# OvO1111/JointImageGeneration

Measured on AMD Instinct MI355X. Metric: sampled voxels/sec @50 DDIM steps, 128^3 mask + 512^2x256 CT, higher is better.
Workload: dtype bf16; 1 GPU; C5 full GuideGen volume per GPU: CCDM 128^3 K=14 250 steps -> LDM 256 slices x (cond-encode + 50 DDIM @4x64x64 + AE decode 512^2); volumes_per_gpu=1, ccdm_steps=250, ddim_steps=50, slices=256, parallelism=replicas x1 (one volume per GPU, no collective), weights=random-init (seed recipe)

## Files before the change

include/guidegen_hip.h:

```cpp
#ifndef GUIDEGEN_HIP_H
#define GUIDEGEN_HIP_H

#include <stdint.h>

#ifdef __cplusplus
extern "C" {
#endif

typedef enum {
    GG_OK = 0,
    GG_ERR_BAD_SHAPE = -1,
    GG_ERR_BAD_DTYPE = -2,
    GG_ERR_UNSUPPORTED = -3,
    GG_ERR_WORKSPACE_TOO_SMALL = -4,
    GG_ERR_HIP = -5
} gg_status;

typedef enum { GG_BF16 = 0, GG_F32 = 1 } gg_dtype;

const char *gg_last_error(void);
int gg_version(void);

typedef struct {
    int32_t N, D, H, W;
// ... 9 lines not shown
    int32_t prologue_act;
    int32_t path_hint;
    const void *src1;
    const void *src2;
    const void *weight;
    const float *bias;
    int64_t bias_stride;
    const void *residual;
    void *out;
    const float *gn_scale;
    const float *gn_shift;
    void *workspace;
    int64_t workspace_bytes;
    void *reserved_ptr;
    int64_t *gn_acc;
    float *ddim_x;
    const float *ddim_scalars;
    float *ddim_pred_x0;
    void *ddim_unet_in;
    int64_t ddim_unet_in_stride;
    int32_t epilogue_geglu;
    int32_t pro_c_logical;
    const int64_t *pro_acc1;
    const int64_t *pro_acc2;
    const float *pro_gamma;
    const float *pro_beta;
    float pro_eps;
    int32_t skip_C1, skip_C2;
    int32_t reserved_tail;
    const void *skip_src1;
    const void *skip_src2;
    const void *skip_weight;
    const int32_t *post_xt;
    int32_t *post_labels_out;
    const float *post_scalars;
    const float *post_E;
    uint64_t post_philox_seed;
    const int64_t *post_philox_offset_dev;
    void *post_onehot_out;
    int64_t post_onehot_stride;
    int32_t post_draw;
    int32_t reserved_tail2;
    const uint64_t *post_philox_seeds;
    int64_t post_rows_per_sample;
} gg_conv_desc;

int64_t gg_conv_packed_weight_bytes(int32_t Cout, int32_t Cin_pad, int32_t ntaps);
int gg_conv_pack_weight(const float *w_f32, int32_t Cout, int32_t Cin, int32_t Cin_pad, int32_t ntaps,
                        void *packed_bf16, void *stream);
int64_t gg_conv_workspace_bytes(const gg_conv_desc *desc);
int gg_conv_fuses_prologue(const gg_conv_desc *desc);
int gg_conv_fuses_posterior(const gg_conv_desc *desc);
int gg_conv_runs_halo_tile(const gg_conv_desc *desc);
int gg_conv_emits_stats(const gg_conv_desc *desc);
int gg_conv_prologue_from_acc(const gg_conv_desc *desc);
int gg_conv_fuses_skip(const gg_conv_desc *desc);
int gg_conv_fuses_ddim(const gg_conv_desc *desc);
int gg_conv_forward(const gg_conv_desc *desc, void *stream);

int64_t gg_groupnorm_workspace_bytes(int32_t N, int64_t S, int32_t C);
int gg_groupnorm_stats(const void *src1, int32_t C1, const void *src2, int32_t C2, int32_t N, int64_t S,
                       int32_t C_logical, const float *gamma, const float *beta, float eps,
                       float *scale_out, float *shift_out, void *workspace, int64_t workspace_bytes, void *stream);
int gg_groupnorm_apply(const void *src1, int32_t C1, const void *src2, int32_t C2, int32_t N, int64_t S,
                       const float *scale, const float *shift, int32_t act, void *out, void *stream);
int gg_groupnorm_fused_supported(int64_t S, int32_t C1, int32_t C2, int32_t C_logical);
int gg_groupnorm_fused(const void *src1, int32_t C1, const void *src2, int32_t C2, int32_t N, int64_t S, int32_t C_logical,
                       const float *gamma, const float *beta, float eps, int32_t act, void *out, void *stream);
int gg_groupnorm_apply_acc(const void *src1, int32_t C1, const int64_t *acc1, const void *src2, int32_t C2, const int64_t *acc2,
                           int32_t N, int64_t S, int32_t C_logical, const float *gamma, const float *beta, float eps,
                           int32_t act, void *out, void *stream);

int gg_groupnorm_scale_shift_acc(const int64_t *acc1, int32_t stripes1, int32_t C1, const int64_t *acc2, int32_t stripes2, int32_t C2,
                                 int32_t N, int64_t S, int32_t C_logical, const float *gamma, const float *beta, float eps,
                                 float *scale_out, float *shift_out, void *stream);

int gg_resample2x(const void *src, int32_t dtype, int32_t N, int32_t D, int32_t H, int32_t W, int32_t C_pad, int32_t C_logical,
                  int32_t resample_d, int32_t mode, const float *scale, const float *shift, int32_t act, void *dst, void *stream);
int gg_film_fold(float *scale, float *shift, int32_t coef_stride, int32_t N, int32_t C, const float *film, int64_t film_stride, void *stream);

typedef struct {
    int32_t N, heads, head_dim;
    int32_t Tq, Tkv;
    int64_t ldq, hsq, ldk, hsk, ldv, hsv, ldo, hso;
    float scale;
    int32_t reserved;
    const void *q, *k, *v;
    void *out;
    void *workspace;
    int64_t workspace_bytes;
} gg_attention_desc;
int gg_attention_forward(const gg_attention_desc *desc, void *stream);
int64_t gg_attention_workspace_bytes(const gg_attention_desc *desc);
int gg_attention_plan(const gg_attention_desc *desc, int32_t plan[4]);

int gg_layernorm(const void *x, int64_t rows, int32_t C, const float *gamma, const float *beta, float eps,
                 void *out, void *stream);
int gg_geglu(const void *h, int64_t rows, int32_t inner, void *out, void *stream);
int gg_add(const void *a, const void *b, int64_t n, void *out, void *stream);

int gg_linear_f32(const float *in, int32_t M, int32_t I, const float *W, const float *b, int32_t O,
                  int32_t act_in, float *out, int64_t out_stride, void *stream);
int gg_timestep_embedding(const float *t, int32_t M, int32_t dim, float max_period, float *out, void *stream);

int gg_nchw_f32_to_cl_bf16(const float *src, int32_t N, int32_t C, int64_t S, void *dst, int32_t C_pad,
                           int32_t c_offset, int32_t zero_fill, void *stream);
// ... 73 lines not shown
```

jointimagegeneration_amd/_lib.py:

```python
from __future__ import annotations

import ctypes as C
import os

_HERE = os.path.dirname(os.path.abspath(__file__))
LIB_PATH = os.path.join(_HERE, "csrc", "libguidegen_hip.so")

GG_BF16, GG_F32 = 0, 1

vp, i32, i64, u64, f32 = C.c_void_p, C.c_int32, C.c_int64, C.c_uint64, C.c_float


class ConvDesc(C.Structure):
    _fields_ = [
        ("N", i32), ("D", i32), ("H", i32), ("W", i32),
        ("C1", i32), ("C2", i32), ("Cout", i32), ("Cout_pad", i32),
        ("kd", i32), ("kh", i32), ("kw", i32), ("stride", i32), ("pad", i32), ("upsample", i32),
        ("Do", i32), ("Ho", i32), ("Wo", i32), ("out_dtype", i32), ("prologue_act", i32), ("path_hint", i32),
        ("src1", vp), ("src2", vp), ("weight", vp), ("bias", vp), ("bias_stride", i64),
        ("residual", vp), ("out", vp), ("gn_scale", vp), ("gn_shift", vp), ("workspace", vp), ("workspace_bytes", i64), ("reserved_ptr", vp), ("gn_acc", vp),
        ("ddim_x", vp), ("ddim_scalars", vp), ("ddim_pred_x0", vp), ("ddim_unet_in", vp), ("ddim_unet_in_stride", i64),
        ("epilogue_geglu", i32), ("pro_c_logical", i32), ("pro_acc1", vp), ("pro_acc2", vp), ("pro_gamma", vp), ("pro_beta", vp),
        ("pro_eps", f32), ("skip_C1", i32), ("skip_C2", i32), ("reserved_tail", i32), ("skip_src1", vp), ("skip_src2", vp), ("skip_weight", vp),
        ("post_xt", vp), ("post_labels_out", vp), ("post_scalars", vp), ("post_E", vp), ("post_philox_seed", C.c_uint64),
        ("post_philox_offset_dev", vp), ("post_onehot_out", vp), ("post_onehot_stride", i64), ("post_draw", i32), ("reserved_tail2", i32),
        ("post_philox_seeds", vp), ("post_rows_per_sample", i64),
    ]


class AttentionDesc(C.Structure):
    _fields_ = [
        ("N", i32), ("heads", i32), ("head_dim", i32), ("Tq", i32), ("Tkv", i32),
        ("ldq", i64), ("hsq", i64), ("ldk", i64), ("hsk", i64), ("ldv", i64), ("hsv", i64), ("ldo", i64), ("hso", i64),
        ("scale", f32), ("reserved", i32),
        ("q", vp), ("k", vp), ("v", vp), ("out", vp), ("workspace", vp), ("workspace_bytes", i64),
    ]


SIGNATURES = {
    "gg_last_error": (C.c_char_p, []),
    "gg_version": (C.c_int, []),
    "gg_conv_packed_weight_bytes": (i64, [i32, i32, i32]),
    "gg_conv_pack_weight": (C.c_int, [vp, i32, i32, i32, i32, vp, vp]),
    "gg_conv_forward": (C.c_int, [C.POINTER(ConvDesc), vp]),
    "gg_conv_workspace_bytes": (i64, [C.POINTER(ConvDesc)]),
    "gg_conv_fuses_prologue": (C.c_int, [C.POINTER(ConvDesc)]),
    "gg_conv_runs_halo_tile": (C.c_int, [C.POINTER(ConvDesc)]),
    "gg_conv_emits_stats": (C.c_int, [C.POINTER(ConvDesc)]),
    "gg_conv_prologue_from_acc": (C.c_int, [C.POINTER(ConvDesc)]),
    "gg_conv_fuses_skip": (C.c_int, [C.POINTER(ConvDesc)]),
    "gg_conv_fuses_ddim": (C.c_int, [C.POINTER(ConvDesc)]),
    "gg_conv_fuses_posterior": (C.c_int, [C.POINTER(ConvDesc)]),
    "gg_groupnorm_workspace_bytes": (i64, [i32, i64, i32]),
    "gg_groupnorm_stats": (C.c_int, [vp, i32, vp, i32, i32, i64, i32, vp, vp, f32, vp, vp, vp, i64, vp]),
    "gg_groupnorm_apply": (C.c_int, [vp, i32, vp, i32, i32, i64, vp, vp, i32, vp, vp]),
    "gg_groupnorm_apply_acc": (C.c_int, [vp, i32, vp, vp, i32, vp, i32, i64, i32, vp, vp, f32, i32, vp, vp]),
    "gg_groupnorm_fused_supported": (C.c_int, [i64, i32, i32, i32]),
    "gg_groupnorm_fused": (C.c_int, [vp, i32, vp, i32, i32, i64, i32, vp, vp, f32, i32, vp, vp]),
    "gg_groupnorm_scale_shift_acc": (C.c_int, [vp, i32, i32, vp, i32, i32, i32, i64, i32, vp, vp, f32, vp, vp, vp]),
    "gg_attention_forward": (C.c_int, [C.POINTER(AttentionDesc), vp]),
    "gg_attention_workspace_bytes": (i64, [C.POINTER(AttentionDesc)]),
    "gg_attention_plan": (C.c_int, [C.POINTER(AttentionDesc), C.POINTER(i32)]),
    "gg_layernorm": (C.c_int, [vp, i64, i32, vp, vp, f32, vp, vp]),
    "gg_geglu": (C.c_int, [vp, i64, i32, vp, vp]),
    "gg_add": (C.c_int, [vp, vp, i64, vp, vp]),
    "gg_linear_f32": (C.c_int, [vp, i32, i32, vp, vp, i32, i32, vp, i64, vp]),
    "gg_timestep_embedding": (C.c_int, [vp, i32, i32, f32, vp, vp]),
    "gg_nchw_f32_to_cl_bf16": (C.c_int, [vp, i32, i32, i64, vp, i32, i32, i32, vp]),
    "gg_cl_to_nchw_f32": (C.c_int, [vp, i32, i32, i32, i64, i32, vp, vp]),
    "gg_ccdm_posterior_sample": (C.c_int, [vp, i32, i32, vp, vp, u64, vp, i32, vp, i32, i64, vp, vp, vp, i32, vp]),
    "gg_ccdm_posterior_sample_seeds": (C.c_int, [vp, i32, i32, vp, vp, vp, i64, vp, i32, vp, i32, i64, vp, vp, vp, i32, vp]),
    "gg_labels_to_onehot": (C.c_int, [vp, i64, i32, vp, i32, vp]),
    "gg_ddim_step": (C.c_int, [vp, vp, i32, vp, vp, i64, i32, vp, vp, i32, vp]),
    "gg_minmax_normalise": (C.c_int, [vp, i64, vp, vp, vp]),
    "gg_ddpm_step": (C.c_int, [vp, vp, i32, vp, vp, i64, i32, vp, i32, vp]),
    "gg_inpaint_blend": (C.c_int, [vp, vp, vp, i32, vp, vp, i64, i32, vp, i32, vp]),
    "gg_vq_nearest": (C.c_int, [vp, i32, vp, i32, i32, i64, vp, vp, i32, vp]),
    "gg_ddim_step_vq": (C.c_int, [vp, vp, i32, vp, vp, i32, vp, i32, i64, i32, vp, vp, vp, i32, vp]),
    "gg_label_confusion": (C.c_int, [vp, i32, vp, i32, i64, i32, vp, vp, vp]),
    "gg_volume_views_cl": (C.c_int, [vp, i32, i32, i32, i32, i32, i64, i64, vp, vp, vp, i32, vp]),
    "gg_relu_cl": (C.c_int, [vp, i32, i64, vp]),
    "gg_lpips_tap_workspace_bytes": (i64, [i32, i32, i32, i32, i32]),
    "gg_lpips_tap": (C.c_int, [vp, vp, i32, i32, i32, i32, i32, vp, vp, vp, vp, vp, i32, vp, i64, vp]),
    "gg_unfold_cl": (C.c_int, [vp, i32, i32, i32, i32, i32, i32, vp, i32, i32, i32, i32, i32, i32, i32, vp]),
    "gg_fold_weighted_cl": (C.c_int, [vp, i32, vp, vp, vp, i32, i32, i32, i32, i32, i32, i32, i32, i32, vp]),
    "gg_lincomb4": (C.c_int, [vp, vp, vp, vp, f32, f32, f32, f32, f32, i64, vp, vp]),
    "gg_conv_forward_f32": (C.c_int, [C.POINTER(ConvDesc), vp]),
    "gg_groupnorm_f32": (C.c_int, [vp, i32, vp, i32, i32, i64, i32, vp, vp, f32, i32, vp, vp, vp]),
    "gg_attention_forward_f32": (C.c_int, [C.POINTER(AttentionDesc), vp]),
    "gg_groupnorm_f32_film": (C.c_int, [vp, i32, i32, i64, i32, vp, vp, f32, vp, i64, i32, vp, vp, vp]),
    "gg_resample2x": (C.c_int, [vp, i32, i32, i32, i32, i32, i32, i32, i32, i32, vp, vp, i32, vp, vp]),
    "gg_film_fold": (C.c_int, [vp, vp, i32, i32, i32, vp, i64, vp]),
    "gg_mask_to_cond_slice": (C.c_int, [vp, i32, i32, i32, i32, i32, i32, i32, i32, vp, vp, i32, vp, vp]),
    "gg_mask_to_cond_slices": (C.c_int, [vp, i32, i32, i32, i32, i32, i32, i32, vp, i32, vp, vp, vp, i32, vp]),
    "gg_minmax_normalise_scatter": (C.c_int, [vp, i32, i64, vp, vp, i32, vp, i32, i32, vp, vp]),
    "gg_ubench_mfma_bf16": (C.c_int, [i32, i32, i32, vp, C.POINTER(C.c_double), vp]),
    "gg_ubench_stream_copy": (C.c_int, [vp, vp, i64, vp]),
}

_lib = None
# ... 27 lines not shown
```

jointimagegeneration_amd/csrc/gg_conv.h:

```cpp
#pragma once
#include "gg_common.h"

struct ConvParams {
    int N, D, H, W, C1, C2, Cout, Cout_pad;
    int kd, kh, kw, stride, pad, upsample;
    int Do, Ho, Wo, out_dtype, prologue_act;
    int path_hint;
    int nchunk1, nchunk, ntaps;
    long long M;
    long long bias_stride;
    const bf16_t *src1, *src2, *weight, *residual;
    const float *bias, *gn_scale, *gn_shift;
    void *out;
    float *ws;
    int splitk;
    long long *gn_acc;
    float *ddim_x, *ddim_pred_x0;
    const float *ddim_scalars;
    bf16_t *ddim_unet_in;
    long long ddim_unet_in_stride;
    unsigned mg_osp, mg_ohw, mg_wo;
    int epi_geglu;
    const long long *pro_acc1, *pro_acc2;
    const float *pro_gamma, *pro_beta;
    float pro_eps;
    int pro_clog;
    const bf16_t *skip_src1, *skip_src2, *skip_weight;
    int skip_C1, skip_C2;
    const int *post_xt;
    int *post_labels_out;
    const float *post_scalars, *post_E;
    unsigned long long post_seed;
    const long long *post_offset_dev;
    bf16_t *post_onehot_out;
    long long post_onehot_stride;
    int post_draw;
    const unsigned long long *post_seeds;
    long long post_rows_per_sample;
};

#define GG_BOX_HINT_GENERIC 10
#define GG_BOX_HINT_SPEC_ONLY 11

#define GG_ACC_SUM_SCALE 268435456.0f
#define GG_ACC_SQ_SCALE 1048576.0f
#ifndef GG_ACC_STRIPES
#define GG_ACC_STRIPES 1
#endif
#define GG_ACC_STRIPES_HALO 32

__device__ __forceinline__ int swz64(int row, int chunk) { return chunk ^ ((row >> 1) & 2); }


__device__ __forceinline__ float gg_row16_sum(float x)
{
    x += __builtin_bit_cast(float, __builtin_amdgcn_mov_dpp(__builtin_bit_cast(int, x), 0xB1, 0xF, 0xF, true));
    x += __builtin_bit_cast(float, __builtin_amdgcn_mov_dpp(__builtin_bit_cast(int, x), 0x4E, 0xF, 0xF, true));
    x += __builtin_bit_cast(float, __builtin_amdgcn_mov_dpp(__builtin_bit_cast(int, x), 0x141, 0xF, 0xF, true));
    x += __builtin_bit_cast(float, __builtin_amdgcn_mov_dpp(__builtin_bit_cast(int, x), 0x140, 0xF, 0xF, true));
    return x;
}
```

jointimagegeneration_amd/csrc/gg_conv.hip:

```cpp
#include "gg_conv.h"
#include <stdlib.h>

template <int NT, int PF, int PRO>
__global__ __launch_bounds__(256) void conv_gather_kernel(const ConvParams p)
{
    constexpr int BM = 128;
    constexpr int XBYTES = BM * 64;
    constexpr int WBYTES = NT * 32 * 64;
    constexpr int STAGE = XBYTES + WBYTES;
    constexpr int WITER = (NT * 128 + 255) / 256;
    __shared__ __attribute__((aligned(16))) char smem[2 * STAGE];

    const int tid = threadIdx.x;
    const int lane = tid & 63;
    const int wave = tid >> 6;
    const long long m0 = (long long)blockIdx.x * BM;
    const int g0 = blockIdx.y * NT;

    const int xq = tid & 3;
    int bn[2], bd[2], bh[2], bw[2];
    bool rv[2];
    const bf16_t *rb1[2], *rb2[2];
    const unsigned osp = (unsigned)(p.Do * p.Ho * p.Wo);
    const unsigned ohw = (unsigned)(p.Ho * p.Wo);
// ... 513 lines not shown
    }
}

__global__ void conv_pack_weight_kernel(const float *__restrict__ w, int Cout, int Cin, int Cin_pad, int ntaps,
                                        int Cout_pad, bf16_t *__restrict__ dst)
{
    const int nchunk = Cin_pad >> 5;
    const long long total = (long long)Cout_pad * ntaps * Cin_pad;
    for (long long i = (long long)blockIdx.x * blockDim.x + threadIdx.x; i < total;
         i += (long long)gridDim.x * blockDim.x) {
        int cil = (int)(i & 31);
        int col = (int)((i >> 5) & 31);
        long long t = i >> 10;
        int chunk = (int)(t % nchunk);
        t /= nchunk;
        int tap = (int)(t % ntaps);
        int g = (int)(t / ntaps);
        int co = g * 32 + col, ci = chunk * 32 + swz64(col, cil >> 3) * 8 + (cil & 7);
        float v = 0.f;
        if (co < Cout && ci < Cin) v = w[((long long)co * Cin + ci) * ntaps + tap];
        dst[i] = (bf16_t)v;
    }
}

extern "C" int64_t gg_conv_packed_weight_bytes(int32_t Cout, int32_t Cin_pad, int32_t ntaps)
{
    int64_t cp = ((int64_t)Cout + 31) / 32 * 32;
    return cp * ntaps * Cin_pad * 2;
}

extern "C" int gg_conv_pack_weight(const float *w, int32_t Cout, int32_t Cin, int32_t Cin_pad, int32_t ntaps,
                                   void *packed, void *stream)
{
    if (Cin_pad % 32 || Cin > Cin_pad || Cout <= 0 || ntaps <= 0) GG_FAIL(GG_ERR_BAD_SHAPE, "pack_weight: bad shape");
    int Cout_pad = (Cout + 31) / 32 * 32;
    long long total = (long long)Cout_pad * ntaps * Cin_pad;
    int blocks = (int)((total + 255) / 256);
    if (blocks > 4096) blocks = 4096;
    hipLaunchKernelGGL(conv_pack_weight_kernel, dim3(blocks), dim3(256), 0, (hipStream_t)stream, w, Cout, Cin, Cin_pad,
                       ntaps, Cout_pad, (bf16_t *)packed);
    GG_CHECK_LAUNCH();
    return GG_OK;
}

int gg_conv_halo_try(const ConvParams &p, hipStream_t stream);
bool gg_conv_halo_prefers_separate_norm(const ConvParams &p);
#ifndef GG_HALO_SEPARATE_NORM
#define GG_HALO_SEPARATE_NORM 1
#endif
int gg_conv_box_try(const ConvParams &p, hipStream_t stream);
bool gg_conv_box_fuses_prologue(const ConvParams &p);
int gg_conv_tiny_plan(long long M, int Cout_pad, int KS, int prologue_act);
int gg_conv_tiny_launch(const ConvParams &p, hipStream_t stream);

static int launch_splitk_reduce(const ConvParams &p, hipStream_t stream, bool cap_blocks)
{
    long long blocks = (p.M * (p.Cout_pad / 4) + 255) / 256;
    if (cap_blocks && blocks > 2048) blocks = 2048;
    hipLaunchKernelGGL(conv_splitk_reduce_kernel, dim3((unsigned)blocks), dim3(256), 0, stream, p);
    GG_CHECK_LAUNCH();
    return GG_OK;
}

template <int NT>
static int launch_gather(const ConvParams &p, hipStream_t stream)
{
    dim3 grid((unsigned)((p.M + 127) / 128), (unsigned)(p.Cout_pad / (32 * NT)), (unsigned)p.splitk);
    if (p.prologue_act)
        hipLaunchKernelGGL((conv_gather_kernel<NT, (NT <= 2 ? 4 : 2), 1>), grid, dim3(256), 0, stream, p);
    else
        hipLaunchKernelGGL((conv_gather_kernel<NT, (NT <= 2 ? 4 : 2), 0>), grid, dim3(256), 0, stream, p);
    GG_CHECK_LAUNCH();
    return p.splitk > 1 ? launch_splitk_reduce(p, stream, true) : GG_OK;
}

static int launch_gather_nt(int NT, const ConvParams &p, hipStream_t stream)
{
    switch (NT) {
        case 5: return launch_gather<5>(p, stream);
        case 4: return launch_gather<4>(p, stream);
        case 3: return launch_gather<3>(p, stream);
        case 2: return launch_gather<2>(p, stream);
        default: return launch_gather<1>(p, stream);
    }
}

struct GatherPlan { int NT, splitk; };
static GatherPlan plan_gather(long long M, int Cout_pad, int KS)
{
    const int G = Cout_pad / 32;
    int NT = (G % 4 == 0) ? 4 : (G % 5 == 0) ? 5 : (G % 3 == 0) ? 3 : (G % 2 == 0) ? 2 : 1;
    const long long mb = (M + 127) / 128;
    int splitk = 1;
    constexpr int k_target = 512, k_minsteps = 8;
    if (mb * (G / NT) < 192) {
        if (G % 2 == 0 && NT > 2 && mb * (G / 2) <= 1024) NT = 2;
        if (mb * (G / NT) < 192 && NT > 1) NT = 1;
        long long blocks = mb * (G / NT);
        long long want = (k_target + blocks - 1) / blocks;
        long long maxs = KS / k_minsteps > 0 ? KS / k_minsteps : 1;
        splitk = (int)(want < maxs ? want : maxs);
        if (splitk < 1) splitk = 1;
        if (splitk > 64) splitk = 64;
    }
    return {NT, splitk};
}

static int plan_gather5(long long M, int C1, int C2, int Cout_pad, int ntaps)
{
    if (C1 % 160 || C2 % 160) return 0;
    const long long blocks = ((M + 63) / 64) * (Cout_pad / 32);
    if (blocks >= 4096) return 0;
    const int KS5 = ((C1 + C2) / 160) * ntaps;
    constexpr int g5_target = 320, g5_minsteps = 5;
    long long sk = (g5_target + blocks - 1) / blocks;
    long long maxs = KS5 / g5_minsteps > 0 ? KS5 / g5_minsteps : 1;
    if (sk > maxs) sk = maxs;
    if (sk < 1) sk = 1;
    if (sk > 32) sk = 32;
    return (int)sk;
}

extern "C" int64_t gg_conv_workspace_bytes(const gg_conv_desc *d)
{
    if (!d || d->epilogue_geglu) return 0;
    long long M = (long long)d->N * d->Do * d->Ho * d->Wo;
    int KS = d->kd * d->kh * d->kw * ((d->C1 + d->C2) / 32);
    if (int tsk = gg_conv_tiny_plan(M, d->Cout_pad, KS, d->prologue_act)) return tsk > 1 ? (int64_t)tsk * M * d->Cout_pad * 4 : 0;
    if (int s5 = plan_gather5(M, d->C1, d->C2, d->Cout_pad, d->kd * d->kh * d->kw)) return s5 > 1 ? (int64_t)s5 * M * d->Cout_pad * 4 : 0;
    GatherPlan pl = plan_gather(M, d->Cout_pad, KS);
    return pl.splitk > 1 ? (int64_t)pl.splitk * M * d->Cout_pad * 4 : 0;
}

static void fill_params(const gg_conv_desc *d, ConvParams &p)
{
    p.N = d->N; p.D = d->D; p.H = d->H; p.W = d->W; p.C1 = d->C1; p.C2 = d->C2; p.Cout = d->Cout; p.Cout_pad = d->Cout_pad;
    p.kd = d->kd; p.kh = d->kh; p.kw = d->kw; p.stride = d->stride; p.pad = d->pad; p.upsample = d->upsample;
    p.Do = d->Do; p.Ho = d->Ho; p.Wo = d->Wo; p.out_dtype = d->out_dtype; p.prologue_act = d->prologue_act; p.path_hint = d->path_hint;
    p.nchunk1 = d->C1 / 32; p.nchunk = (d->C1 + d->C2) / 32; p.ntaps = d->kd * d->kh * d->kw;
    p.M = (long long)d->N * d->Do * d->Ho * d->Wo;
    p.bias_stride = d->bias_stride;
    p.src1 = (const bf16_t *)d->src1; p.src2 = (const bf16_t *)d->src2; p.weight = (const bf16_t *)d->weight;
    p.residual = (const bf16_t *)d->residual; p.bias = d->bias; p.gn_scale = d->gn_scale; p.gn_shift = d->gn_shift;
    p.out = d->out;
    p.ws = nullptr;
    p.splitk = 1;
    p.gn_acc = (long long *)d->gn_acc;
    p.ddim_x = d->ddim_x; p.ddim_pred_x0 = d->ddim_pred_x0; p.ddim_scalars = d->ddim_scalars;
    p.ddim_unet_in = (bf16_t *)d->ddim_unet_in; p.ddim_unet_in_stride = d->ddim_unet_in_stride;
    p.epi_geglu = d->epilogue_geglu;
    p.pro_acc1 = (const long long *)d->pro_acc1; p.pro_acc2 = (const long long *)d->pro_acc2; p.pro_gamma = d->pro_gamma; p.pro_beta = d->pro_beta;
    p.pro_eps = d->pro_eps; p.pro_clog = d->pro_c_logical;
    if (d->gn_scale || d->gn_shift || !d->prologue_act) p.pro_acc1 = p.pro_acc2 = nullptr;
    p.skip_src1 = (const bf16_t *)d->skip_src1; p.skip_src2 = (const bf16_t *)d->skip_src2; p.skip_weight = (const bf16_t *)d->skip_weight;
    p.skip_C1 = d->skip_C1; p.skip_C2 = d->skip_C2;
    p.post_xt = d->post_xt; p.post_labels_out = d->post_labels_out; p.post_scalars = d->post_scalars; p.post_E = d->post_E;
    p.post_seed = d->post_philox_seed; p.post_offset_dev = (const long long *)d->post_philox_offset_dev;
    p.post_onehot_out = (bf16_t *)d->post_onehot_out; p.post_onehot_stride = d->post_onehot_stride; p.post_draw = d->post_draw;
    p.post_seeds = (const unsigned long long *)d->post_philox_seeds; p.post_rows_per_sample = d->post_rows_per_sample;
    p.mg_osp = gg_magic_u32(p.M, d->Do * d->Ho * d->Wo); p.mg_ohw = gg_magic_u32(p.M, d->Ho * d->Wo); p.mg_wo = gg_magic_u32(p.M, d->Wo);
}

static bool halo_try_dry(const ConvParams &p) { return gg_conv_halo_try(p, (hipStream_t)-1) == GG_OK; }
static bool box_try_dry(const ConvParams &p) { return gg_conv_box_try(p, (hipStream_t)-1) == GG_OK; }
static bool desc_channels_ok(const gg_conv_desc *d) { return d && d->C1 > 0 && d->C1 % 32 == 0 && d->C2 % 32 == 0 && d->Cout_pad % 32 == 0; }

static int take_splitk_workspace(const gg_conv_desc *d, ConvParams &p, int splitk)
{
    if (splitk > 1) {
        const long long need = (long long)splitk * p.M * p.Cout_pad * 4;
        if (!d->workspace || d->workspace_bytes < need)
            GG_FAIL(GG_ERR_WORKSPACE_TOO_SMALL, "conv: split-K needs %lld workspace bytes (gg_conv_workspace_bytes), got %lld", need, (long long)d->workspace_bytes);
        p.ws = (float *)d->workspace;
    }
    p.splitk = splitk;
    return GG_OK;
}

extern "C" int gg_conv_runs_halo_tile(const gg_conv_desc *d)
{
    if (!desc_channels_ok(d) || d->epilogue_geglu) return 0;
    ConvParams p;
    fill_params(d, p);
    return halo_try_dry(p) ? 1 : 0;
}

extern "C" int gg_conv_fuses_prologue(const gg_conv_desc *d)
{
    if (!desc_channels_ok(d) || d->epilogue_geglu) return 0;
    ConvParams p;
    fill_params(d, p);
    if (halo_try_dry(p)) return (GG_HALO_SEPARATE_NORM && d->path_hint == 0 && gg_conv_halo_prefers_separate_norm(p)) ? 0 : 1;
    if (box_try_dry(p)) return gg_conv_box_fuses_prologue(p) ? 1 : 0;
    return 0;
}

bool gg_conv_box_emits_stats(const ConvParams &p);
bool gg_conv_box_prologue_from_acc(const ConvParams &p);
bool gg_conv_halo_fuses_posterior(const ConvParams &p);

extern "C" int gg_conv_fuses_posterior(const gg_conv_desc *d)
{
    if (!desc_channels_ok(d) || d->epilogue_geglu || d->residual || d->out_dtype != GG_F32 || d->gn_acc ||
        d->ddim_x || d->skip_C1) return 0;
    ConvParams p;
    fill_params(d, p);
    return gg_conv_halo_fuses_posterior(p) ? 1 : 0;
}

extern "C" int gg_conv_prologue_from_acc(const gg_conv_desc *d)
{
    if (!desc_channels_ok(d) || d->epilogue_geglu || !d->prologue_act) return 0;
    if (d->pro_c_logical <= 0 || d->pro_c_logical % 32 || d->pro_c_logical > d->C1 + d->C2 || (d->C2 && d->pro_c_logical < d->C1)) return 0;
    ConvParams p;
    fill_params(d, p);
    if (halo_try_dry(p)) return 0;
    return box_try_dry(p) && gg_conv_box_prologue_from_acc(p) ? 1 : 0;
}

extern "C" int gg_conv_fuses_skip(const gg_conv_desc *d)
{
    if (!desc_channels_ok(d) || d->epilogue_geglu || d->skip_C1 <= 0 || d->skip_C1 % 32 || d->skip_C2 % 32 ||
        d->skip_C2 < 0 || d->residual || d->ddim_x)
        return 0;
    ConvParams p;
    fill_params(d, p);
    if (halo_try_dry(p)) return 0;
    return box_try_dry(p) ? 1 : 0;
}

extern "C" int gg_conv_fuses_ddim(const gg_conv_desc *d)
{
    if (!desc_channels_ok(d) || d->out_dtype != GG_F32 || d->Cout != 4 || d->residual) return 0;
    ConvParams p;
    fill_params(d, p);
    if (halo_try_dry(p)) return 0;
    return box_try_dry(p) ? 1 : 0;
}


extern "C" int gg_conv_emits_stats(const gg_conv_desc *d)
{
    if (!desc_channels_ok(d) || d->out_dtype != GG_BF16 || d->epilogue_geglu) return 0;
    ConvParams p;
    fill_params(d, p);
    if (halo_try_dry(p)) return GG_ACC_STRIPES_HALO;
    if (box_try_dry(p)) return gg_conv_box_emits_stats(p) ? GG_ACC_STRIPES : 0;
    if (gg_conv_tiny_plan(p.M, p.Cout_pad, p.ntaps * p.nchunk, p.prologue_act)) return 0;
    const long long osp = (long long)d->Do * d->Ho * d->Wo;
    return (plan_gather5(p.M, p.C1, p.C2, p.Cout_pad, p.ntaps) == 1 && osp % 64 == 0) ? GG_ACC_STRIPES : 0;
}

#ifdef GG_EXP_WPREFETCH
__global__ __launch_bounds__(256) void exp_wprefetch_kernel(const u32x4 *w, long long n16, unsigned *sink)
{
    unsigned a = 0;
    if (n16 <= (3 << 20) / 16 * 1) {
        for (long long i = (long long)(blockIdx.x >> 3) * 256 + threadIdx.x; i < n16; i += 32 * 256) { const u32x4 v = w[i]; a ^= v[0] ^ v[1] ^ v[2] ^ v[3]; }
    } else
    for (long long i = (long long)blockIdx.x * 256 + threadIdx.x; i < n16; i += 256 * 256) { const u32x4 v = w[i]; a ^= v[0] ^ v[1] ^ v[2] ^ v[3]; }
    if (a == 0x12345679u) sink[0] = a;
}
#endif
extern "C" int gg_conv_forward(const gg_conv_desc *d, void *stream_)
{
    hipStream_t stream = (hipStream_t)stream_;
    if (!d) GG_FAIL(GG_ERR_BAD_SHAPE, "conv: null desc");
    if (d->C1 <= 0 || d->C1 % 32 || d->C2 % 32 || d->C2 < 0) GG_FAIL(GG_ERR_BAD_SHAPE, "conv: C1/C2 must be multiples of 32 (got %d, %d)", d->C1, d->C2);
    if (d->Cout_pad % 32 || d->Cout > d->Cout_pad || d->Cout <= 0) GG_FAIL(GG_ERR_BAD_SHAPE, "conv: bad Cout/Cout_pad %d/%d", d->Cout, d->Cout_pad);
    auto okk = [](int k) { return k == 1 || k == 3; };
    if (!okk(d->kd) || !okk(d->kh) || !okk(d->kw)) GG_FAIL(GG_ERR_UNSUPPORTED, "conv: kernel extent must be 1 or 3");
    if (d->stride != 1 && d->stride != 2) GG_FAIL(GG_ERR_UNSUPPORTED, "conv: stride must be 1 or 2");
    if (d->upsample && d->stride != 1) GG_FAIL(GG_ERR_UNSUPPORTED, "conv: upsample with stride");
    if (d->out_dtype != GG_BF16 && d->out_dtype != GG_F32) GG_FAIL(GG_ERR_BAD_DTYPE, "conv: out dtype");
    if (!d->src1 || !d->weight || (!d->out && !d->post_xt) || (d->C2 && !d->src2)) GG_FAIL(GG_ERR_BAD_SHAPE, "conv: null pointer");
    if (d->post_xt) {
        if (!gg_conv_fuses_posterior(d)) GG_FAIL(GG_ERR_UNSUPPORTED, "conv: this shape cannot run the fused CCDM reverse step (gg_conv_fuses_posterior)");
        if (!d->post_labels_out || !d->post_scalars) GG_FAIL(GG_ERR_BAD_SHAPE, "conv: fused CCDM reverse step needs labels_out and scalars");
        if (d->post_onehot_out && (d->post_onehot_stride < d->Cout || (d->post_onehot_stride & 1) || ((uintptr_t)d->post_onehot_out & 3)))
            GG_FAIL(GG_ERR_BAD_SHAPE, "conv: fused CCDM reverse step: one-hot rows must be 4-byte aligned (even stride >= K)");
        if (d->post_philox_seeds && d->post_rows_per_sample != (int64_t)d->Do * d->Ho * d->Wo)
            GG_FAIL(GG_ERR_BAD_SHAPE, "conv: fused CCDM reverse step: post_rows_per_sample %lld must be Do*Ho*Wo = %lld",
                    (long long)d->post_rows_per_sample, (long long)d->Do * d->Ho * d->Wo);
    }
    const bool pro_acc = d->prologue_act && !d->gn_scale && !d->gn_shift && d->pro_acc1;
    if (pro_acc) {
        if (!gg_conv_prologue_from_acc(d)) GG_FAIL(GG_ERR_UNSUPPORTED, "conv: this shape cannot compute its GroupNorm prologue from accumulators (gg_conv_prologue_from_acc)");
        if (!d->pro_gamma || !d->pro_beta || (d->C2 && !d->pro_acc2)) GG_FAIL(GG_ERR_BAD_SHAPE, "conv: accumulator prologue needs gamma / beta and one accumulator per source");
    } else if (d->prologue_act && (!d->gn_scale || !d->gn_shift)) GG_FAIL(GG_ERR_BAD_SHAPE, "conv: prologue without scale/shift");
    if (d->N <= 0 || d->D <= 0 || d->H <= 0 || d->W <= 0 || d->Do <= 0 || d->Ho <= 0 || d->Wo <= 0) GG_FAIL(GG_ERR_BAD_SHAPE, "conv: empty extent");
    auto expect = [&](int in, int k, int up) {
        int e = up ? in * 2 : in;
        if (k == 1) return (d->upsample && !up) ? e : (e - 1) / d->stride + 1;
        return (d->stride == 1) ? e + 2 * d->pad - 2 : (d->pad == 1 ? (e + 2 - 3) / 2 + 1 : (e + 1 - 3) / 2 + 1);
    };
    const int upD = d->upsample && d->kd == 3, upHW = d->upsample;
    if (d->Do != expect(d->D, d->kd, upD) || d->Ho != expect(d->H, d->kh, upHW) || d->Wo != expect(d->W, d->kw, upHW))
        GG_FAIL(GG_ERR_BAD_SHAPE, "conv: output extent (%d,%d,%d) inconsistent with input (%d,%d,%d) k=(%d,%d,%d) stride %d pad %d up %d",
                d->Do, d->Ho, d->Wo, d->D, d->H, d->W, d->kd, d->kh, d->kw, d->stride, d->pad, d->upsample);

    if (d->skip_C1) {
        if (!gg_conv_fuses_skip(d)) GG_FAIL(GG_ERR_UNSUPPORTED, "conv: this shape cannot take a K-concatenated skip projection (gg_conv_fuses_skip)");
        if (!d->skip_src1 || !d->skip_weight || (d->skip_C2 && !d->skip_src2)) GG_FAIL(GG_ERR_BAD_SHAPE, "conv: skip projection without source / weight");
// ... 4 lines not shown
    fill_params(d, p);
    if (p.M >= (1LL << 31) || (long long)d->D * d->H * d->W * (d->C1 > d->C2 ? d->C1 : d->C2) >= (1LL << 31))
        GG_FAIL(GG_ERR_UNSUPPORTED, "conv: tensor too large for 32-bit in-sample offsets");

    if (d->epilogue_geglu) {
        if (d->kd != 1 || d->kh != 1 || d->kw != 1 || d->stride != 1 || d->upsample || d->residual || d->out_dtype != GG_BF16 || d->gn_acc ||
            d->ddim_x || d->Cout % 32 || d->bias_stride)
            GG_FAIL(GG_ERR_UNSUPPORTED, "conv: the GEGLU epilogue needs a 1x1 conv, bf16 output, Cout = 2*inner with inner %% 16 == 0, a shared bias, no residual / gn_acc / ddim");
        return launch_gather_nt(plan_gather(p.M, p.Cout_pad, p.ntaps * p.nchunk).NT, p, stream);
    }
#ifdef GG_EXP_WPREFETCH
    {
        const long long wbytes = (long long)(p.Cout_pad / 32) * p.ntaps * p.nchunk * 2048;
        hipLaunchKernelGGL(exp_wprefetch_kernel, dim3(256), dim3(256), 0, stream, (const u32x4 *)p.weight, wbytes >> 4, (unsigned *)d->out);
    }
#endif
#ifdef GG_H3_STAMPS
    if (d->path_hint == 7 && d->workspace) p.ws = (float *)d->workspace;
#endif
    int rc = gg_conv_halo_try(p, stream);
#ifdef GG_H3_STAMPS
    p.ws = nullptr;
#endif
    if (rc != GG_ERR_UNSUPPORTED) return rc;
    if (d->post_xt) GG_FAIL(GG_ERR_UNSUPPORTED, "conv: the halo-tile kernel did not take this shape, and no other kernel runs the fused CCDM reverse step");
#ifdef GG_BOX_STAMPS
    if (d->path_hint == 98) p.ws = (float *)d->workspace;
#endif
    rc = gg_conv_box_try(p, stream);
#ifdef GG_BOX_STAMPS
    p.ws = nullptr;
#endif
    if (rc != GG_ERR_UNSUPPORTED) return rc;

    if (int tsk = gg_conv_tiny_plan(p.M, p.Cout_pad, p.ntaps * p.nchunk, p.prologue_act)) {
        if ((rc = take_splitk_workspace(d, p, tsk)) != GG_OK) return rc;
        rc = gg_conv_tiny_launch(p, stream);
        if (rc != GG_OK || tsk == 1) return rc;
        return launch_splitk_reduce(p, stream, false);
    }

    if (int s5 = plan_gather5(p.M, p.C1, p.C2, p.Cout_pad, p.ntaps)) {
        if ((rc = take_splitk_workspace(d, p, s5)) != GG_OK) return rc;
        dim3 grid((unsigned)((p.M + 63) / 64), (unsigned)(p.Cout_pad / 32), (unsigned)s5);
        if (p.prologue_act && (((long long)p.Do * p.Ho * p.Wo) % 64 || p.C1 + p.C2 > 2560))
            GG_FAIL(GG_ERR_UNSUPPORTED, "conv: fused prologue on the 160-step kernel needs Do*Ho*Wo %% 64 == 0 and C <= 2560");
        if (p.prologue_act) hipLaunchKernelGGL(conv_gather5_kernel<1>, grid, dim3(256), 0, stream, p);
        else hipLaunchKernelGGL(conv_gather5_kernel<0>, grid, dim3(256), 0, stream, p);
        GG_CHECK_LAUNCH();
        return s5 > 1 ? launch_splitk_reduce(p, stream, true) : GG_OK;
    }

    GatherPlan pl = plan_gather(p.M, p.Cout_pad, p.ntaps * p.nchunk);
    if ((rc = take_splitk_workspace(d, p, pl.splitk)) != GG_OK) return rc;
    return launch_gather_nt(pl.NT, p, stream);
}
```

jointimagegeneration_amd/ops.py:

```python
from __future__ import annotations

import ctypes as C
from dataclasses import dataclass
from typing import Optional, Sequence, Tuple

import torch

from . import _lib
from ._lib import GG_BF16, GG_F32, AttentionDesc, ConvDesc, check


def _stream() -> int:
    return torch.cuda.current_stream().cuda_stream


def _ptr(t: Optional[torch.Tensor]) -> Optional[int]:
    return None if t is None else t.data_ptr()


def require_gpu(t: torch.Tensor, what: str) -> None:
    if not t.is_cuda:
        raise RuntimeError(f"{what}: tensor is on {t.device}; the GuideGen engine runs on MI355X only "
                           "(no CPU fallback; the CPU restatement lives in oracle/ and is test infrastructure)")

# ... 139 lines not shown
            out.append((s - 1) // stride + 1)
        else:
            e = s * 2 if upsample else s
            if stride == 1:
                out.append(e + 2 * pad - 2)
            else:
                out.append((e + 2 - 3) // 2 + 1 if pad == 1 else (e + 1 - 3) // 2 + 1)
    return tuple(out)


def _shape_desc(src1: CL, cout: int, k, stride: int, pad: int, upsample: bool, src2: Optional[CL]) -> "ConvDesc":
    N, D, H, W, C1 = src1.t.shape
    Do, Ho, Wo = conv_out_extent((D, H, W), k, stride, pad, upsample)
    d = ConvDesc()
    d.N, d.D, d.H, d.W = N, D, H, W
    d.C1, d.C2 = C1, (src2.t.shape[-1] if src2 is not None else 0)
    d.Cout, d.Cout_pad = cout, pad32(cout)
    d.kd, d.kh, d.kw = k
    d.stride, d.pad, d.upsample = stride, pad, 1 if upsample else 0
    d.Do, d.Ho, d.Wo = Do, Ho, Wo
    d.path_hint = PATH_HINT
    return d


def conv_prologue_from_acc(src1: CL, cout: int, act: bool, k=(1, 3, 3), stride: int = 1, pad: int = 1, upsample: bool = False,
                           src2: Optional[CL] = None, **_ignored) -> bool:
    if not PROLOGUE_FROM_ACC or is_f32(src1.t) or not has_stats(src1, src2):
        return False
    if src2 is not None and src1.C != src1.Cpad:
        return False
    d = _shape_desc(src1, cout, k, stride, pad, upsample, src2)
    d.prologue_act = 1 if act else 2
    d.pro_c_logical = src1.C + (src2.C if src2 is not None else 0)
    return bool(_lib.load().gg_conv_prologue_from_acc(C.byref(d)))


SKIP_KCONCAT = True


def conv_fuses_skip(src1: CL, cout: int, skip1: CL, skip2: Optional[CL] = None, k=(1, 3, 3), stride: int = 1, pad: int = 1, upsample: bool = False,
                    **_ignored) -> bool:
    if not SKIP_KCONCAT or is_f32(src1.t) or (skip2 is not None and skip1.C != skip1.Cpad):
        return False
    d = _shape_desc(src1, cout, k, stride, pad, upsample, None)
    d.skip_C1, d.skip_C2 = skip1.Cpad, (skip2.Cpad if skip2 is not None else 0)
    return bool(_lib.load().gg_conv_fuses_skip(C.byref(d)))


def conv_runs_halo_tile(src1: CL, cout: int, k=(1, 3, 3), stride: int = 1, pad: int = 1, upsample: bool = False,
                        src2: Optional[CL] = None, **_ignored) -> bool:
    if is_f32(src1.t):
        return False
    return bool(_lib.load().gg_conv_runs_halo_tile(C.byref(_shape_desc(src1, cout, k, stride, pad, upsample, src2))))


def conv_fuses_prologue(src1: CL, cout: int, k=(1, 3, 3), stride: int = 1, pad: int = 1, upsample: bool = False,
                        src2: Optional[CL] = None, **_ignored) -> bool:
    if is_f32(src1.t):
        return False
    return bool(_lib.load().gg_conv_fuses_prologue(C.byref(_shape_desc(src1, cout, k, stride, pad, upsample, src2))))


GN_ACC = True
TINY_IMAGE_POSITIONS = 0
FUSE_POSTERIOR = True
PROLOGUE_FROM_ACC = True
GN_ACC_MAX_ELEMS = 1 << 21
GN_ACC_MIN_ELEMS = 1 << 17
_ARENA_ENTRIES = 1 << 19
_ARENAS = {}


def stats_begin(device) -> None:
    if not GN_ACC:
        return
    a = _ARENAS.get(str(device))
    if a is None:
        a = _ARENAS[str(device)] = dict(buf=torch.zeros(_ARENA_ENTRIES, dtype=torch.int64, device=device), off=0, hi=0, active=False)
    else:
        a["hi"] = max(a["hi"], a["off"])
    if torch.cuda.is_current_stream_capturing():
        a["buf"].zero_()
        a["hi"] = _ARENA_ENTRIES
    elif a["hi"]:
        a["buf"][:min(_ARENA_ENTRIES, (a["hi"] + 65535) // 65536 * 65536)].zero_()
    a["off"] = 0
    a["active"] = True


def stats_end(device) -> None:
    a = _ARENAS.get(str(device))
    if a is not None:
        a["hi"] = max(a["hi"], a["off"])
        a["active"] = False


def _stats_alloc(device, N: int, cp: int, stripes: int) -> Optional[torch.Tensor]:
    a = _ARENAS.get(str(device))
    n = N * stripes * cp * 2
    if a is None or not a["active"] or a["off"] + n > _ARENA_ENTRIES:
        return None
    v = a["buf"][a["off"]:a["off"] + n].view(N, stripes, cp, 2)
    a["off"] += n
    return v


# ... 614 lines not shown
```

Measured before the change: 804,300 voxels/s.

## Add persistent LDS-resident-weight kernel for 1x1 bf16 convolutions

Adds a specialised 1x1 convolution kernel for bf16 layers that would otherwise take the single-pass gather path. Each block keeps its slice of the weights in LDS for its whole lifetime and strides over row runs persistently, prefetching the next run's input rows into registers while the MFMAs for the current run execute. It targets the per-tile weight reloads and generic gather indexing overhead of 1x1 convs such as skip projections and proj_in/proj_out. A parent-only path hint and a dry-run query let callers opt out, and only selected channel counts are instantiated.

```diff
diff --git a/include/guidegen_hip.h b/include/guidegen_hip.h
--- a/include/guidegen_hip.h
+++ b/include/guidegen_hip.h
@@ -85,6 +85,7 @@
 int gg_conv_fuses_prologue(const gg_conv_desc *desc);
 int gg_conv_fuses_posterior(const gg_conv_desc *desc);
 int gg_conv_runs_halo_tile(const gg_conv_desc *desc);
+int gg_conv_runs_rows1x1(const gg_conv_desc *desc);
 int gg_conv_emits_stats(const gg_conv_desc *desc);
 int gg_conv_prologue_from_acc(const gg_conv_desc *desc);
 int gg_conv_fuses_skip(const gg_conv_desc *desc);
diff --git a/jointimagegeneration_amd/_lib.py b/jointimagegeneration_amd/_lib.py
--- a/jointimagegeneration_amd/_lib.py
+++ b/jointimagegeneration_amd/_lib.py
@@ -46,6 +46,7 @@
     "gg_conv_workspace_bytes": (i64, [C.POINTER(ConvDesc)]),
     "gg_conv_fuses_prologue": (C.c_int, [C.POINTER(ConvDesc)]),
     "gg_conv_runs_halo_tile": (C.c_int, [C.POINTER(ConvDesc)]),
+    "gg_conv_runs_rows1x1": (C.c_int, [C.POINTER(ConvDesc)]),
     "gg_conv_emits_stats": (C.c_int, [C.POINTER(ConvDesc)]),
     "gg_conv_prologue_from_acc": (C.c_int, [C.POINTER(ConvDesc)]),
     "gg_conv_fuses_skip": (C.c_int, [C.POINTER(ConvDesc)]),
diff --git a/jointimagegeneration_amd/csrc/gg_conv.h b/jointimagegeneration_amd/csrc/gg_conv.h
--- a/jointimagegeneration_amd/csrc/gg_conv.h
+++ b/jointimagegeneration_amd/csrc/gg_conv.h
@@ -6,6 +6,7 @@
     int kd, kh, kw, stride, pad, upsample;
     int Do, Ho, Wo, out_dtype, prologue_act;
     int path_hint;
+    int parent_only;
     int nchunk1, nchunk, ntaps;
     long long M;
     long long bias_stride;
@@ -42,6 +43,8 @@
 #define GG_BOX_HINT_GENERIC 10
 #define GG_BOX_HINT_SPEC_ONLY 11
 
+#define GG_CONV_HINT_PARENT 12
+
 #define GG_ACC_SUM_SCALE 268435456.0f
 #define GG_ACC_SQ_SCALE 1048576.0f
 #ifndef GG_ACC_STRIPES
diff --git a/jointimagegeneration_amd/csrc/gg_conv.hip b/jointimagegeneration_amd/csrc/gg_conv.hip
--- a/jointimagegeneration_amd/csrc/gg_conv.hip
+++ b/jointimagegeneration_amd/csrc/gg_conv.hip
@@ -589,6 +589,7 @@
 bool gg_conv_box_fuses_prologue(const ConvParams &p);
 int gg_conv_tiny_plan(long long M, int Cout_pad, int KS, int prologue_act);
 int gg_conv_tiny_launch(const ConvParams &p, hipStream_t stream);
+int gg_conv_rows1x1_try(const ConvParams &p, hipStream_t stream);
 
 static int launch_splitk_reduce(const ConvParams &p, hipStream_t stream, bool cap_blocks)
 {
@@ -673,7 +674,8 @@
 {
     p.N = d->N; p.D = d->D; p.H = d->H; p.W = d->W; p.C1 = d->C1; p.C2 = d->C2; p.Cout = d->Cout; p.Cout_pad = d->Cout_pad;
     p.kd = d->kd; p.kh = d->kh; p.kw = d->kw; p.stride = d->stride; p.pad = d->pad; p.upsample = d->upsample;
-    p.Do = d->Do; p.Ho = d->Ho; p.Wo = d->Wo; p.out_dtype = d->out_dtype; p.prologue_act = d->prologue_act; p.path_hint = d->path_hint;
+    p.Do = d->Do; p.Ho = d->Ho; p.Wo = d->Wo; p.out_dtype = d->out_dtype; p.prologue_act = d->prologue_act;
+    p.parent_only = d->path_hint == GG_CONV_HINT_PARENT; p.path_hint = p.parent_only ? 0 : d->path_hint;
     p.nchunk1 = d->C1 / 32; p.nchunk = (d->C1 + d->C2) / 32; p.ntaps = d->kd * d->kh * d->kw;
     p.M = (long long)d->N * d->Do * d->Ho * d->Wo;
     p.bias_stride = d->bias_stride;
@@ -727,7 +729,7 @@
     if (!desc_channels_ok(d) || d->epilogue_geglu) return 0;
     ConvParams p;
     fill_params(d, p);
-    if (halo_try_dry(p)) return (GG_HALO_SEPARATE_NORM && d->path_hint == 0 && gg_conv_halo_prefers_separate_norm(p)) ? 0 : 1;
+    if (halo_try_dry(p)) return (GG_HALO_SEPARATE_NORM && p.path_hint == 0 && gg_conv_halo_prefers_separate_norm(p)) ? 0 : 1;
     if (box_try_dry(p)) return gg_conv_box_fuses_prologue(p) ? 1 : 0;
     return 0;
 }
@@ -786,6 +788,22 @@
     if (gg_conv_tiny_plan(p.M, p.Cout_pad, p.ntaps * p.nchunk, p.prologue_act)) return 0;
     const long long osp = (long long)d->Do * d->Ho * d->Wo;
     return (plan_gather5(p.M, p.C1, p.C2, p.Cout_pad, p.ntaps) == 1 && osp % 64 == 0) ? GG_ACC_STRIPES : 0;
+}
+
+static bool reaches_single_pass_gather(const gg_conv_desc *d, ConvParams &p)
+{
+    if (!desc_channels_ok(d) || d->epilogue_geglu || d->C2 < 0) return false;
+    fill_params(d, p);
+    if (halo_try_dry(p) || box_try_dry(p) || gg_conv_tiny_plan(p.M, p.Cout_pad, p.ntaps * p.nchunk, p.prologue_act) ||
+        plan_gather5(p.M, p.C1, p.C2, p.Cout_pad, p.ntaps))
+        return false;
+    return plan_gather(p.M, p.Cout_pad, p.ntaps * p.nchunk).splitk == 1;
+}
+
+extern "C" int gg_conv_runs_rows1x1(const gg_conv_desc *d)
+{
+    ConvParams p;
+    return reaches_single_pass_gather(d, p) && gg_conv_rows1x1_try(p, (hipStream_t)-1) == GG_OK ? 1 : 0;
 }
 
 #ifdef GG_EXP_WPREFETCH
@@ -896,6 +914,7 @@
     }
 
     GatherPlan pl = plan_gather(p.M, p.Cout_pad, p.ntaps * p.nchunk);
+    if (pl.splitk == 1 && (rc = gg_conv_rows1x1_try(p, stream)) != GG_ERR_UNSUPPORTED) return rc;
     if ((rc = take_splitk_workspace(d, p, pl.splitk)) != GG_OK) return rc;
     return launch_gather_nt(pl.NT, p, stream);
 }
diff --git a/jointimagegeneration_amd/csrc/gg_conv_rows.hip b/jointimagegeneration_amd/csrc/gg_conv_rows.hip
--- /dev/null
+++ b/jointimagegeneration_amd/csrc/gg_conv_rows.hip
@@ -0,0 +1,199 @@
+#include "gg_conv.h"
+#include <atomic>
+
+#define GG_ROWS_CST(PT) ((PT) * 1024 + 64)
+
+template <int NCH, int NT, int PT>
+__global__ __launch_bounds__(256) void conv_rows1x1_kernel(const ConvParams p, const int nruns)
+{
+    constexpr int WB = NT * NCH * 2048;
+    constexpr int CST = GG_ROWS_CST(PT);
+    constexpr int XW = NCH * CST;
+    constexpr int J = PT * NCH;
+    constexpr int RUN = 64 * PT;
+    extern __shared__ __attribute__((aligned(16))) char smem[];
+
+    const int tid = threadIdx.x, lane = tid & 63;
+    const int wave = __builtin_amdgcn_readfirstlane(tid >> 6);
+    const int fr = lane & 15, fq = lane >> 4;
+    const int g0 = blockIdx.y * NT;
+    char *xw = smem + WB + wave * XW;
+
+    {
+        const u32x4 *wsrc = reinterpret_cast<const u32x4 *>(p.weight + (long long)g0 * NCH * 1024);
+        for (int i = tid; i < WB / 16; i += 256) *reinterpret_cast<u32x4 *>(smem + i * 16) = wsrc[i];
+    }
+
+    const int J1 = PT * p.nchunk1;
+    const int P1 = p.nchunk1 * 4, P2 = (NCH - p.nchunk1) * 4;
+    const unsigned mg1 = (1u << 20) / (unsigned)P1 + 1u;
+    const unsigned mg2 = P2 ? (1u << 20) / (unsigned)P2 + 1u : 0u;
+    int xrow[J], xlds[J];
+#pragma unroll
+    for (int j = 0; j < J; ++j) {
+        const bool second = j >= J1;
+        const unsigned i = (unsigned)((second ? j - J1 : j) * 64 + lane);
+        const unsigned row = (i * (second ? mg2 : mg1)) >> 20;
+        const unsigned q = i - row * (unsigned)(second ? P2 : P1);
+        const int chunk = (second ? p.nchunk1 : 0) + (int)(q >> 2);
+        xrow[j] = (int)row;
+        xlds[j] = chunk * CST + (int)row * 64 + swz64((int)row, (int)(q & 3)) * 16;
+    }
+
+    u32x4 xr[J];
+    auto load_rows = [&](int run) {
+        const long long mw = (long long)run * RUN + wave * (16 * PT);
+        const u32x4 *s1 = reinterpret_cast<const u32x4 *>(p.src1 + mw * p.C1);
+        const u32x4 *s2 = p.src2 ? reinterpret_cast<const u32x4 *>(p.src2 + mw * p.C2) : nullptr;
+#pragma unroll
+        for (int j = 0; j < J; ++j) {
+            u32x4 v = {0u, 0u, 0u, 0u};
+            if (mw + xrow[j] < p.M) v = (j >= J1) ? s2[(j - J1) * 64 + lane] : s1[j * 64 + lane];
+            xr[j] = v;
+        }
+    };
+
+    const unsigned osp = (unsigned)(p.Do * p.Ho * p.Wo);
+    int run = blockIdx.x;
+    if (run < nruns) load_rows(run);
+    __syncthreads();
+
+    for (; run < nruns; run += gridDim.x) {
+        __builtin_amdgcn_fence(__ATOMIC_RELEASE, "wavefront");
+        __builtin_amdgcn_wave_barrier();
+#pragma unroll
+        for (int j = 0; j < J; ++j) *reinterpret_cast<u32x4 *>(xw + xlds[j]) = xr[j];
+        __builtin_amdgcn_fence(__ATOMIC_RELEASE, "wavefront");
+        __builtin_amdgcn_wave_barrier();
+        __builtin_amdgcn_fence(__ATOMIC_ACQUIRE, "wavefront");
+
+        const long long mw = (long long)run * RUN + wave * (16 * PT);
+        f32x4 bv[PT][2 * NT];
+        bf16x4 resv[PT][2 * NT];
+#pragma unroll
+        for (int pt = 0; pt < PT; ++pt) {
+            const long long m = mw + pt * 16 + fr;
+            const long long mc = m < p.M ? m : p.M - 1;
+            const int n = p.N == 1 ? 0 : (int)((unsigned)mc / osp);
+            const float *brow = p.bias ? p.bias + (long long)n * p.bias_stride : nullptr;
+#pragma unroll
+            for (int ct = 0; ct < 2 * NT; ++ct) {
+                const int co = (g0 * 32) + ct * 16 + fq * 4;
+                bv[pt][ct] = brow ? *reinterpret_cast<const f32x4 *>(brow + co) : f32x4{0.f, 0.f, 0.f, 0.f};
+                if (p.residual) resv[pt][ct] = *reinterpret_cast<const bf16x4 *>(p.residual + mc * p.Cout_pad + co);
+            }
+        }
+        if (run + (int)gridDim.x < nruns) load_rows(run + (int)gridDim.x);
+
+        f32x4 acc[PT][2 * NT];
+#pragma unroll
+        for (int a = 0; a < PT; ++a)
+#pragma unroll
+            for (int b = 0; b < 2 * NT; ++b) acc[a][b] = f32x4{0.f, 0.f, 0.f, 0.f};
+#pragma unroll
+        for (int c = 0; c < NCH; ++c) {
+            bf16x8 xf[PT];
+#pragma unroll
+            for (int pt = 0; pt < PT; ++pt) {
+                const int r = pt * 16 + fr;
+                xf[pt] = *reinterpret_cast<const bf16x8 *>(xw + c * CST + r * 64 + swz64(r, fq) * 16);
+            }
+#pragma unroll
+            for (int ct = 0; ct < 2 * NT; ++ct) {
+                const int r = (ct & 1) * 16 + fr;
+                const bf16x8 wf = *reinterpret_cast<const bf16x8 *>(smem + ((ct >> 1) * NCH + c) * 2048 + r * 64 + swz64(r, fq) * 16);
+#pragma unroll
+                for (int pt = 0; pt < PT; ++pt)
+                    acc[pt][ct] = __builtin_amdgcn_mfma_f32_16x16x32_bf16(wf, xf[pt], acc[pt][ct], 0, 0, 0);
+            }
+        }
+
+#pragma unroll
+        for (int pt = 0; pt < PT; ++pt) {
+            const long long m = mw + pt * 16 + fr;
+            if (m >= p.M) continue;
+#pragma unroll
+            for (int ct = 0; ct < 2 * NT; ++ct) {
+                const int co = (g0 * 32) + ct * 16 + fq * 4;
+                f32x4 v = acc[pt][ct];
+                if (p.bias) v += bv[pt][ct];
+                if (p.residual) {
+                    const bf16x4 r = resv[pt][ct];
+#pragma unroll
+                    for (int j = 0; j < 4; ++j) v[j] += (float)r[j];
+                }
+#pragma unroll
+                for (int j = 0; j < 4; ++j)
+                    if (co + j >= p.Cout) v[j] = 0.f;
+                bf16x4 ob;
+#pragma unroll
+                for (int j = 0; j < 4; ++j) ob[j] = (bf16_t)v[j];
+                *reinterpret_cast<bf16x4 *>((bf16_t *)p.out + m * p.Cout_pad + co) = ob;
+            }
+        }
+    }
+}
+
+struct RowsPlan { int NCH, NT, PT, lds; };
+static constexpr int k_rows_lds_max = 80 * 1024;
+static constexpr int k_rows_cus = 256;
+static int rows_lds_bytes(int NCH, int NT, int PT) { return NT * NCH * 2048 + 4 * NCH * GG_ROWS_CST(PT); }
+
+static bool plan_rows1x1(const ConvParams &p, RowsPlan &pl)
+{
+    const int NCH = p.nchunk, G = p.Cout_pad / 32;
+    if (NCH != 2 && NCH != 4 && NCH != 6 && NCH != 8) return false;
+    if (NCH < 8 && p.M < (1 << 18)) return false;
+    if (G % 2) return false;
+    int NT = (G % 4 == 0) ? 4 : 2;
+    int PT = ((p.M + 127) / 128) * (G / NT) >= k_rows_cus ? 2 : 1;
+    while (rows_lds_bytes(NCH, NT, PT) > k_rows_lds_max || (NCH == 4 && NT == 4 && PT == 2)) {
+        if (NT == 4) NT = 2;
+        else if (PT == 2) PT = 1;
+        else return false;
+    }
+    pl = {NCH, NT, PT, rows_lds_bytes(NCH, NT, PT)};
+    return true;
+}
+
+template <int NCH, int NT, int PT>
+static int launch_rows1x1(const ConvParams &p, const RowsPlan &pl, int dev, hipStream_t stream)
+{
+    static std::atomic<unsigned long long> attr_mask{0};
+    const unsigned long long dev_bit = 1ull << (dev & 63);
+    if (!(attr_mask.load(std::memory_order_acquire) & dev_bit)) {
+        if (hipFuncSetAttribute((const void *)conv_rows1x1_kernel<NCH, NT, PT>, hipFuncAttributeMaxDynamicSharedMemorySize, pl.lds) != hipSuccess)
+            GG_FAIL(GG_ERR_HIP, "conv: rows1x1 kernel: %d bytes of LDS refused", pl.lds);
+        attr_mask.fetch_or(dev_bit, std::memory_order_release);
+    }
+    const long long nruns = (p.M + 64 * PT - 1) / (64 * PT);
+    const int ctiles = p.Cout_pad / (32 * NT);
+    long long gx = ((long long)k_rows_cus * 2 + ctiles - 1) / ctiles;
+    if (gx > nruns) gx = nruns;
+    if (gx < 1) gx = 1;
+    hipLaunchKernelGGL((conv_rows1x1_kernel<NCH, NT, PT>), dim3((unsigned)gx, (unsigned)ctiles), dim3(256), pl.lds, stream, p, (int)nruns);
+    GG_CHECK_LAUNCH();
+    return GG_OK;
+}
+
+int gg_conv_rows1x1_try(const ConvParams &p, hipStream_t stream)
+{
+    if (p.ntaps != 1 || p.stride != 1 || p.upsample || p.prologue_act || p.out_dtype != GG_BF16) return GG_ERR_UNSUPPORTED;
+    if (p.gn_acc || p.epi_geglu || p.skip_C1 || p.ddim_x || p.post_xt || p.splitk != 1) return GG_ERR_UNSUPPORTED;
+    if (p.parent_only || p.M < 4096) return GG_ERR_UNSUPPORTED;
+    RowsPlan pl;
+    if (!plan_rows1x1(p, pl)) return GG_ERR_UNSUPPORTED;
+    if (stream == (hipStream_t)-1) return GG_OK;
+    int dev = 0;
+    if (hipGetDevice(&dev) != hipSuccess) GG_FAIL(GG_ERR_HIP, "conv: rows1x1 kernel: no device");
+#define GG_ROWS_CASE(NCH_, NT_, PT_) \
+    if (pl.NCH == NCH_ && pl.NT == NT_ && pl.PT == PT_) return launch_rows1x1<NCH_, NT_, PT_>(p, pl, dev, stream);
+#define GG_ROWS_NCH(NCH_) GG_ROWS_CASE(NCH_, 2, 1) GG_ROWS_CASE(NCH_, 2, 2) GG_ROWS_CASE(NCH_, 4, 1) GG_ROWS_CASE(NCH_, 4, 2)
+    GG_ROWS_NCH(2)
+    GG_ROWS_CASE(4, 2, 1) GG_ROWS_CASE(4, 2, 2) GG_ROWS_CASE(4, 4, 1)
+    GG_ROWS_CASE(6, 2, 1) GG_ROWS_CASE(6, 2, 2) GG_ROWS_CASE(6, 4, 1)
+    GG_ROWS_CASE(8, 2, 1)
+#undef GG_ROWS_NCH
+#undef GG_ROWS_CASE
+    GG_FAIL(GG_ERR_BAD_SHAPE, "conv: rows1x1 kernel: plan (%d chunks, NT %d, PT %d) is not instantiated", pl.NCH, pl.NT, pl.PT);
+}
diff --git a/jointimagegeneration_amd/ops.py b/jointimagegeneration_amd/ops.py
--- a/jointimagegeneration_amd/ops.py
+++ b/jointimagegeneration_amd/ops.py
@@ -215,6 +215,13 @@
     if is_f32(src1.t):
         return False
     return bool(_lib.load().gg_conv_runs_halo_tile(C.byref(_shape_desc(src1, cout, k, stride, pad, upsample, src2))))
+
+
+def conv_runs_rows1x1(src1: CL, cout: int, k=(1, 1, 1), stride: int = 1, pad: int = 0, upsample: bool = False,
+                      src2: Optional[CL] = None, **_ignored) -> bool:
+    if is_f32(src1.t):
+        return False
+    return bool(_lib.load().gg_conv_runs_rows1x1(C.byref(_shape_desc(src1, cout, k, stride, pad, upsample, src2))))
 
 
 def conv_fuses_prologue(src1: CL, cout: int, k=(1, 3, 3), stride: int = 1, pad: int = 1, upsample: bool = False,
```

After: 808,900 voxels/s (median of 2 runs). No clear change (+0.6%).
